# aszepieniec/stark-anatomy

Hardware: AMD Instinct MI355X
Metric: ntt_field_elements_per_sec (higher is better)
Workload: dtype u128; 1 GPU; ntt_fwd_inv_2^20_1gpu; log2n=20, parallelism=single, passes_per_transform=2

## Files before the change

stark-anatomy_amd/csrc/core.h:

```cpp
#pragma once
#include <hip/hip_runtime.h>
#include <dlfcn.h>
#include <cstdio>
#include <cstdlib>
#include <cstring>
#include <algorithm>
#include <atomic>
#include <chrono>
#include <cerrno>
#include <thread>
#include <sys/random.h>
#include <deque>
#include <functional>
#include <future>
#include <map>
#include <mutex>
#include <string>
#include <tuple>
#include <vector>

#pragma GCC visibility push(default)
#include "../../include/starkcore.h"
#pragma GCC visibility pop
#include "ntt_plan.h"
// ... 40 lines not shown
    void* p = nullptr;
    size_t bytes = 0;
};

struct PlanKey {
    int logn;
    uint64_t lo, hi;
    bool operator<(const PlanKey& o) const { return std::tie(logn, lo, hi) < std::tie(o.logn, o.lo, o.hi); }
};
struct PlanTables {
    Fe* mt = nullptr;
    int mt_log = 0;
    Fe* tl = nullptr;
    Fe* th = nullptr;
    Fe* th_ninv = nullptr;
    struct Direct { int logA, logR; bool scaled; Fe* d; };
    std::vector<Direct> direct;
    uint64_t last_use = 0;
};
struct OuterKey {
    uint64_t lo, hi, order, len, batch, col_base;
    int ninv;
    bool operator<(const OuterKey& o) const { return std::tie(lo, hi, order, len, batch, col_base, ninv) < std::tie(o.lo, o.hi, o.order, o.len, o.batch, o.col_base, o.ninv); }
};
struct OuterTable {
    Fe* d = nullptr;
    uint64_t last_use = 0;
};
struct PowKey {
    uint64_t lo, hi, hi_count;
    bool operator<(const PowKey& o) const { return std::tie(lo, hi, hi_count) < std::tie(o.lo, o.hi, o.hi_count); }
// ... 3 lines not shown
    Fe* hi = nullptr;
    uint64_t last_use = 0;
};

struct Ctx {
    bool init = false;
    int device = -1;
    hipStream_t stream = nullptr;
    std::string err;
    NttTuning tuning;
    std::map<PlanKey, PlanTables> plans;
    std::map<PowKey, PowTables> pows;
    std::map<OuterKey, OuterTable> outers;
    uint64_t tick = 0;
    bool foreign_streams = false;
    int small_divisor_direct = 1;
    std::vector<hipStream_t> seen_streams;
    DevBuf scratch[8];
    std::map<hipStream_t, DevBuf> ntt_work;
    int num_cus = 256;
    int xcd_remap = 1;
    int fixed_shapes = 1;
    int prio_balance = -1;
    int wave_local = 1;
    unsigned long long* trace = nullptr;
    int forest_four_lane_wgs = 256;
    int merkle_big_nlev = 2;
    int fri_tail = -1;
    int fri_tail_stall = -1;
    size_t verify_stage_bytes = 64ull << 20;
// ... 17 lines not shown
        hipError_t _e = (expr);                                                                               \
        if (_e != hipSuccess) return fail(SC_ERR_HIP, std::string(#expr) + ": " + hipGetErrorString(_e));     \
    } while (0)

#define SCCHK(expr)              \
    do {                         \
        int _rc = (expr);        \
        if (_rc != SC_OK) return _rc; \
    } while (0)

struct NttOpts {
    uint64_t in_limit = ~0ull;
    const PowTables* coset = nullptr;
    uint32_t cols = 1;
    uint64_t col_stride_in = 0;
};

constexpr uint64_t FUSE_MAX_W = 1ull << 17;

enum BuildMode { BUILD_SYNC = 0, BUILD_ASYNC = 1, BUILD_NOROOT = 2 };

extern Ctx g;
extern std::mutex g_mu;
extern hipStream_t g_comm_stream_for_free;
extern std::future<void> g_rand_worker;
extern size_t g_rand_prefetched;
extern std::multimap<size_t, void*> g_pool;
extern size_t g_pool_bytes, g_pool_cap;
extern std::deque<PendingFree> g_pending;
extern std::vector<hipEvent_t> g_event_pool;

void reap_pending(bool block);
hipError_t pool_alloc(void** p, size_t bytes);
void pool_free(void* p, size_t bytes);
void pool_clear();
hipEvent_t event_get();
int fail(int code, const std::string& msg);
int ensure_init();
int grow_buffer(DevBuf& b, size_t bytes, void** out);
inline int scratch(int slot, size_t bytes, void** out) { return grow_buffer(g.scratch[slot], bytes, out); }
int check_root(Fe root, uint64_t n);
int build_pow_table(Fe** out, uint64_t count, Fe base_m, uint64_t step, Fe scale_m, hipStream_t st);
void free_plans();
int evict_outer_tables();
int get_plan(Fe root, int logn, bool need_ninv, hipStream_t st, PlanTables** out);
inline NttTables tables_of(const PlanTables& t) {
    NttTables tb;
    tb.mt = t.mt; tb.mt_log = t.mt_log; tb.tl = t.tl; tb.th = t.th;
    return tb;
}
int get_pow(Fe base, uint64_t count, hipStream_t st, PowTables** out);
int plan_batched_direct(NttPlanDesc& d, BatchKind kind, int loglen, int logbatch, PlanTables* pt, const Fe* in, Fe* work, Fe* out, BatchExtras ex, hipStream_t st, bool* ok);
int run_plan(NttPlanDesc& d, hipStream_t st);
int ntt_device(const Fe* d_in, Fe* d_out, int logn, Fe root, bool inverse_scale, const NttOpts& o, hipStream_t st);
Fe root_inverse(Fe root, uint64_t n);
int ntt_any(const Fe* d_in, Fe* d_out, uint64_t n, Fe root, bool inverse, const NttOpts& o, hipStream_t st);
int upload(void* d, const void* h, size_t bytes, hipStream_t st);
int download(void* h, const void* d, size_t bytes, hipStream_t st);
int pointwise_div_device(const Fe* a, const Fe* b, Fe* out, uint64_t n, hipStream_t st);
int pointwise_div_enqueue(const Fe* a, const Fe* b, Fe* out, uint64_t n, hipStream_t st, uint32_t* flag);
int gather_device(const Fe* v, const uint64_t* d_idx, uint64_t k, Fe* d_out, hipStream_t st);
int read_small_polled(const void* d_src, size_t bytes, hipStream_t st, void* host_out);

int merkle_climb(uint64_t* levels, uint64_t N, int lvl, hipStream_t st, volatile uint64_t* host = nullptr, uint64_t seq = 0, bool* published = nullptr);
int merkle_finish(uint64_t* levels, uint64_t width, hipStream_t st);
int root_slot_get();
int merkle_build_device(const Fe* d_elems, uint64_t N, uint8_t root_out[64], sc_merkle** tree, hipStream_t st, BuildMode mode = BUILD_SYNC, const FoldIn* fold = nullptr);
int merkle_root_wait(sc_merkle* t, bool from_free = false);
// ... 82 lines not shown
```

stark-anatomy_amd/csrc/core.hip:

```cpp
#include "core.h"


template <int LOGE> struct PassThreads { static constexpr int value = LOGE >= 4 ? 256 : (LOGE == 3 ? 512 : 1024); };

template <int LOGE>
__global__ void __launch_bounds__(PassThreads<LOGE>::value) ntt_pass_kernel(const PassParams P, uint32_t ntiles, int xcd_remap) {
    extern __shared__ __attribute__((aligned(16))) unsigned char smem_raw[];
    Fe* lds = reinterpret_cast<Fe*>(smem_raw);
    uint32_t wg = blockIdx.x, colbits = 0;
    if (P.col_enable) { colbits = (wg >> P.col_tiles_log) << P.col_tiles_log; wg -= colbits; }
    uint32_t tile = wg;
    if (xcd_remap) tile = (wg & 7u) * (ntiles >> 3) + (wg >> 3);
    tile |= colbits;
    Fe* tw = lds + (1u << (P.logR + P.logC));
    tile_twiddles_to_lds(P, P.logR, threadIdx.x, blockDim.x, tw);
    __syncthreads();
    const int nrounds = (P.logR + LOGE - 1) / LOGE;
    int sh = P.logR;
    for (int r = 0; r < nrounds; ++r) {
        const int s = (r == 0) ? (P.logR - LOGE * (nrounds - 1)) : LOGE;
        sh -= s;
        ntt_round_dispatch<LOGE>(P, s, sh, r == 0, tile, threadIdx.x, lds, tw);
        if (r + 1 < nrounds) __syncthreads();
    }
// ... 381 lines not shown
    return SC_OK;
}

int build_pow_table(Fe** out, uint64_t count, Fe base_m, uint64_t step, Fe scale_m, hipStream_t st) {
    if (count == 0) count = 1;
    HIPCHK(hipMalloc((void**)out, count * sizeof(Fe)));
    unsigned blocks = (unsigned)((count + 255) / 256);
    hipLaunchKernelGGL(pow_table_kernel, dim3(blocks), dim3(256), 0, st, *out, count, base_m, step, scale_m);
    HIPCHK(hipGetLastError());
    return SC_OK;
}

void free_plan_tables(PlanTables& t) {
    hipFree(t.mt); hipFree(t.tl); hipFree(t.th);
    if (t.th_ninv) hipFree(t.th_ninv);
    for (const PlanTables::Direct& e : t.direct) hipFree(e.d);
}

void free_plans() {
    for (auto& kv : g.plans) free_plan_tables(kv.second);
    g.plans.clear();
    for (auto& kv : g.pows) { hipFree(kv.second.lo); hipFree(kv.second.hi); }
    g.pows.clear();
    for (auto& kv : g.outers) hipFree(kv.second.d);
    g.outers.clear();
}

constexpr uint64_t PIN_WINDOW = 64;
constexpr size_t PLAN_CAP = 256, POW_CAP = 64;

template <class Map, class FreeFn>
int evict_tables(Map& m, size_t cap, FreeFn free_entry) {
    if (m.size() < cap) return SC_OK;
    std::vector<std::pair<uint64_t, typename Map::iterator>> old;
    for (auto it = m.begin(); it != m.end(); ++it)
        if (it->second.last_use + PIN_WINDOW < g.tick) old.emplace_back(it->second.last_use, it);
    if (old.empty()) return SC_OK;
    std::sort(old.begin(), old.end(), [](const auto& a, const auto& b) { return a.first < b.first; });
    size_t drop = cap / 4 ? cap / 4 : 1;
    if (drop > old.size()) drop = old.size();
    HIPCHK(hipDeviceSynchronize());
    for (size_t i = 0; i < drop; ++i) { free_entry(old[i].second->second); m.erase(old[i].second); }
    return SC_OK;
}

int get_plan(Fe root, int logn, bool need_ninv, hipStream_t st, PlanTables** out) {
    PlanKey key{logn, root.lo, root.hi};
    auto it = g.plans.find(key);
    bool built = false;
    ++g.tick;
    if (it == g.plans.end()) {
        SCCHK(evict_tables(g.plans, PLAN_CAP, free_plan_tables));
        const uint64_t n = 1ull << logn;
        Fe rm = to_mont(root);
        const TableSizes sz = table_sizes(logn);
        PlanTables t;
        t.mt_log = sz.mt_log;
        SCCHK(build_pow_table(&t.mt, sz.mt, rm, n >> sz.mt_log, fe_mont_one(), st));
        SCCHK(build_pow_table(&t.tl, sz.tl, rm, 1, fe_mont_one(), st));
        SCCHK(build_pow_table(&t.th, sz.th, rm, 4096, fe_mont_one(), st));
        it = g.plans.emplace(key, t).first;
        built = true;
    }
    if (need_ninv && !it->second.th_ninv) {
        const uint64_t n = 1ull << logn;
        Fe ninv_m = mont_inv(to_mont(Fe{n, 0}));
        SCCHK(build_pow_table(&it->second.th_ninv, table_sizes(logn).th, to_mont(root), 4096, ninv_m, st));
        built = true;
    }
    if (built) HIPCHK(hipStreamSynchronize(st));
    it->second.last_use = g.tick;
    *out = &it->second;
    return SC_OK;
}

int get_pow(Fe base, uint64_t count, hipStream_t st, PowTables** out) {
    uint64_t hi_count = (count >> 12) + 1;
    uint64_t hc = 1; while (hc < hi_count) hc <<= 1;
    PowKey key{base.lo, base.hi, hc};
    auto it = g.pows.find(key);
    ++g.tick;
    if (it == g.pows.end()) {
        SCCHK(evict_tables(g.pows, POW_CAP, [](PowTables& t) { hipFree(t.lo); hipFree(t.hi); }));
        Fe bm = to_mont(base);
        PowTables t;
        SCCHK(build_pow_table(&t.lo, 4096, bm, 1, fe_mont_one(), st));
        SCCHK(build_pow_table(&t.hi, hc, bm, 4096, fe_mont_one(), st));
        HIPCHK(hipStreamSynchronize(st));
        it = g.pows.emplace(key, t).first;
    }
    it->second.last_use = g.tick;
    *out = &it->second;
    return SC_OK;
}

int direct_twiddles(PlanTables* pt, const NttPlanDesc& d, int i, bool scaled, hipStream_t st, const Fe** out) {
    const DirectTable t = direct_table(d, i, scaled);
    *out = nullptr;
    if (t.logR + t.logB > g.tuning.direct_tw_max_log) return SC_OK;
    for (const PlanTables::Direct& e : pt->direct)
        if (e.logA == t.logA && e.logR == t.logR && e.scaled == t.scaled) { *out = e.d; return SC_OK; }
    const uint64_t count = 1ull << (t.logR + t.logB);
    Fe* p;
    HIPCHK(hipMalloc((void**)&p, count * sizeof(Fe)));
    pt->direct.push_back({t.logA, t.logR, t.scaled, p});
    hipLaunchKernelGGL(twiddle_table_kernel, dim3((unsigned)((count + 255) / 256)), dim3(256), 0, st, p, t.logB, count, 1ull << t.logA,
                       pt->tl, t.scaled ? pt->th_ninv : pt->th);
    HIPCHK(hipGetLastError());
    HIPCHK(hipStreamSynchronize(st));
    *out = p;
    return SC_OK;
}

int plan_batched_direct(NttPlanDesc& d, BatchKind kind, int loglen, int logbatch, PlanTables* pt, const Fe* in, Fe* work, Fe* out, BatchExtras ex, hipStream_t st, bool* ok) {
    const NttTables tb = tables_of(*pt);
    *ok = plan_batched(d, kind, loglen, logbatch, tb, in, work, out, g.tuning, ex);
    if (!*ok || d.npasses != 2) return SC_OK;
    SCCHK(direct_twiddles(pt, d, 0, false, st, &ex.inner_twd));
    if (ex.inner_twd) *ok = plan_batched(d, kind, loglen, logbatch, tb, in, work, out, g.tuning, ex);
    return SC_OK;
}

template <int LOGE>
void launch_pass(const NttPassDesc& pd, hipStream_t st) {
    int remap = (g.xcd_remap && pd.ntiles >= 16 && (pd.ntiles & 7u) == 0) ? 1 : 0;
    const PassKernel k = pass_kernel(pd, g.fixed_shapes != 0);
    if constexpr (LOGE == 2) {
        if (k.kind == PK_FIXED4) {
            const int lr = pd.p.logR, lc = pd.p.logC;
#define SC_LAUNCH_FIXED(LR, LC, TR, ALT) \
    hipLaunchKernelGGL((ntt_pass_kernel_fixed<2, LR, LC, TR, ALT>), dim3(pd.ntiles * pd.cols), dim3(pd.threads), pd.lds_bytes, st, pd.p, pd.ntiles, remap, g.wave_local)
#define SC_FIXED(LR, LC)                                                          \
            if (lr == LR && lc == LC) {                                           \
// ... 24 lines not shown
        d.pass[i].p.trace = g.trace ? g.trace + trace_off : nullptr;
        trace_off += (size_t)d.pass[i].ntiles * d.pass[i].cols * (d.pass[i].threads >> 6) * TRACE_STAMPS;
        switch (d.pass[i].loge) {
            case 1: launch_pass<1>(d.pass[i], st); break;
            case 2: launch_pass<2>(d.pass[i], st); break;
            case 3: launch_pass<3>(d.pass[i], st); break;
            case 4: launch_pass<4>(d.pass[i], st); break;
            default: return fail(SC_ERR_UNSUPPORTED, "bad loge");
        }
        HIPCHK(hipGetLastError());
    }
    return SC_OK;
}

int ntt_device(const Fe* d_in, Fe* d_out, int logn, Fe root, bool inverse_scale, const NttOpts& o, hipStream_t st) {
    PlanTables* pt;
    SCCHK(get_plan(root, logn, inverse_scale, st, &pt));
    const uint64_t n = 1ull << logn;
    const int m = plan_num_passes(logn, g.tuning);
    NttTables tb = tables_of(*pt);
    tb.th_scaled = (inverse_scale && m > 1) ? pt->th_ninv : nullptr;
    NttIo io;
    io.in = d_in; io.out = d_out; io.in_limit = o.in_limit; io.cols = o.cols; io.col_stride_in = o.col_stride_in;
    if (m > 1) { void* w; SCCHK(grow_buffer(g.ntt_work[st], n * o.cols * sizeof(Fe), &w)); io.work = (Fe*)w; }
    if (o.coset) { io.ol = o.coset->lo; io.oh = o.coset->hi; }
    if (inverse_scale && m == 1) { io.scale_last = true; io.scale = mont_inv(to_mont(Fe{n, 0})); }
    NttPlanDesc d;
    if (!plan_ntt(d, logn, tb, io, g.tuning)) return fail(SC_ERR_UNSUPPORTED, "unsupported transform length");
    if (d.npasses > 1) {
        bool any = false;
        for (int i = 0; i + 1 < d.npasses; ++i) {
            SCCHK(direct_twiddles(pt, d, i, inverse_scale, st, &tb.twd[i]));
            any |= tb.twd[i] != nullptr;
        }
        if (any && !plan_ntt(d, logn, tb, io, g.tuning)) return fail(SC_ERR_UNSUPPORTED, "unsupported transform length");
    }
    return run_plan(d, st);
}

Fe root_inverse(Fe root, uint64_t n) {
    return from_mont(mont_pow(to_mont(root), n - 1));
}

int ntt_any(const Fe* d_in, Fe* d_out, uint64_t n, Fe root, bool inverse, const NttOpts& o, hipStream_t st) {
    if (n <= 1) {
        if (n == 1 && d_in != d_out) HIPCHK(hipMemcpyAsync(d_out, d_in, sizeof(Fe), hipMemcpyDeviceToDevice, st));
        return SC_OK;
// ... 225 lines not shown
    else if (k == "min_tiles_log") g.tuning.min_tiles_log = value;
    else if (k == "single_pass_max_log") g.tuning.single_pass_max_log = value;
    else if (k == "max_digit_log") g.tuning.max_digit_log = value;
    else if (k == "direct_tw_max_log") g.tuning.direct_tw_max_log = value;
    else if (k == "xcd_remap") g.xcd_remap = value;
    else if (k == "fixed_shapes") g.fixed_shapes = value;
    else if (k == "wave_local") g.wave_local = value;
    else if (k == "prio_balance") g.prio_balance = value;
    else if (k == "loge_cols") g.tuning.loge_cols = value;
    else if (k == "tw_on_load") g.tuning.tw_on_load = value;
    else if (k == "prune") g.tuning.prune = value;
    else if (k == "merkle_big_nlev") g.merkle_big_nlev = value < 0 ? 0 : (value > 8 ? 8 : value);
    else if (k == "forest_four_lane_wgs") g.forest_four_lane_wgs = value < 0 ? 0 : value;
    else if (k == "fri_tail") g.fri_tail = value ? 1 : 0;
    else if (k == "small_divisor_direct") g.small_divisor_direct = value ? 1 : 0;
    else if (k == "verify_stage_kb") g.verify_stage_bytes = (size_t)(value < 16 ? 16 : value) << 10;
    else if (k == "fri_tail_stall") g.fri_tail_stall = value;
    else if (k == "pool_cap_mb") g_pool_cap = (size_t)(value < 0 ? 0 : value) << 20;
    else if (k == "pool_trim") {
        if (g.init) { (void)hipDeviceSynchronize(); reap_pending(true); pool_clear(); }
    }
    else return fail(SC_ERR_BAD_ARG, "unknown tuning key " + k);
    return SC_OK;
}

int sc_ntt_num_passes(uint64_t n) {
    std::lock_guard<std::mutex> lk(g_mu);
    if (n < 2 || !is_pow2(n)) return 0;
    return plan_num_passes(ilog2(n), g.tuning);
}
// ... 383 lines not shown
    SCCHK(get_pow(fe_from(factor), rows * row_len, st, &pw));
    const uint64_t cnt = rows * cols;
    hipLaunchKernelGGL(scale_slab_kernel, dim3((unsigned)((cnt + 255) / 256)), dim3(256), 0, st, (const Fe*)d_in, (Fe*)d_out, rows, ilog2(cols), row_len, col_base, pw->lo, pw->hi);
    HIPCHK(hipGetLastError());
    return SC_OK;
}

int sc_poly_mul(const void* a, uint64_t na, const void* b, uint64_t nb, const uint64_t root[2], uint64_t order, void* out, uint64_t n_out) {
    std::lock_guard<std::mutex> lk(g_mu);
    SCCHK(ensure_init());
    if (!is_pow2(order) || order < 2) return fail(SC_ERR_NOT_POW2, "cannot compute ntt of non-power-of-two sequence");
    if (na > order || nb > order || n_out > order || na == 0 || nb == 0) return fail(SC_ERR_BAD_ARG, "operand longer than the transform order");
    Fe rt = fe_from(root);
    SCCHK(check_root(rt, order));
    hipStream_t st = g.stream;
    void *da, *db, *dc;
    SCCHK(scratch(1, order * sizeof(Fe), &da));
    SCCHK(scratch(2, order * sizeof(Fe), &db));
    SCCHK(scratch(3, order * sizeof(Fe), &dc));
    const int logn = ilog2(order);
    NttOpts o;
    SCCHK(upload(dc, a, na * sizeof(Fe), st));
    o.in_limit = na;
    SCCHK(ntt_device((const Fe*)dc, (Fe*)da, logn, rt, false, o, st));
    SCCHK(upload(dc, b, nb * sizeof(Fe), st));
    o.in_limit = nb;
    SCCHK(ntt_device((const Fe*)dc, (Fe*)db, logn, rt, false, o, st));
    hipLaunchKernelGGL(pointwise_mul_kernel, dim3((unsigned)((order + 255) / 256)), dim3(256), 0, st, (const Fe*)da, (const Fe*)db, (Fe*)dc, order);
    HIPCHK(hipGetLastError());
    SCCHK(ntt_device((const Fe*)dc, (Fe*)da, logn, root_inverse(rt, order), true, NttOpts{}, st));
    return download(out, da, n_out * sizeof(Fe), st);
}

static int coset_divide_core(const Fe* d_a, uint64_t na, const Fe* d_b, uint64_t nb, Fe off, Fe rt, uint64_t order, Fe** full, hipStream_t st, uint32_t* zero_flag = nullptr) {
    void *da, *db, *dc;
// ... 217 lines not shown
```

stark-anatomy_amd/csrc/fourstep.hip:

```cpp
#include "core.h"

__global__ void __launch_bounds__(256) outer_table_kernel(Fe* out, uint64_t count, int logcols, uint64_t col_base, const Fe* __restrict__ tl, const Fe* __restrict__ th) {
    uint64_t i = (uint64_t)blockIdx.x * blockDim.x + threadIdx.x;
    if (i >= count) return;
    uint64_t r = i >> logcols, c = i & ((1ull << logcols) - 1);
    out[i] = pow2level(tl, th, r * (col_base + c));
}

__global__ void __launch_bounds__(256) twiddle_matrix_kernel(Fe* __restrict__ data, uint64_t rows, int logcols, uint64_t row_base, uint64_t col_base,
                                                             const Fe* __restrict__ tl, const Fe* __restrict__ th, int scale_enable, Fe scale_m) {
    uint64_t i = (uint64_t)blockIdx.x * blockDim.x + threadIdx.x;
    if (i >= (rows << logcols)) return;
    uint64_t r = i >> logcols, c = i & ((1ull << logcols) - 1);
    uint64_t e = (row_base + r) * (col_base + c);
    Fe t = pow2level(tl, th, e);
    if (scale_enable) t = mont_mul(t, scale_m);
    data[i] = mont_mul(data[i], t);
}

extern "C" {

struct BatchCall {
    const Fe* in = nullptr;
    Fe* out = nullptr;
// ... 35 lines not shown
    ex.diag_lo = c.diag_lo;
    ex.diag_n = c.diag_n;
    ex.block_out = c.block_out;
    ex.block_rows = c.block_rows;
    if (c.out_ld) {
        if (kind != 1 || c.out_ld < batch) return fail(SC_ERR_BAD_ARG, "an output leading dimension belongs to kind 1 and must be >= batch");
        ex.out_ld = c.out_ld;
    }
    if (c.outer) {
        const uint64_t outer_order = c.outer_order, outer_col_base = c.outer_col_base;
        if (!is_pow2(outer_order) || outer_order < len * batch) return fail(SC_ERR_BAD_ARG, "outer twiddle order too small");
        if ((len - 1) * (outer_col_base + batch - 1) >= outer_order) return fail(SC_ERR_BAD_ARG, "outer twiddle exponent out of range");
        Fe ort = c.outer_root;
        if (!c.roots_checked) SCCHK(check_root(ort, outer_order));
        PlanTables* po;
        SCCHK(get_plan(ort, ilog2(outer_order), c.outer_ninv, st, &po));
        ex.outer_tl = po->tl;
        ex.outer_th = c.outer_ninv ? po->th_ninv : po->th;
        ex.outer_col_base = outer_col_base;
        if (g.tuning.direct_tw_max_log > 0 && len * batch <= (1ull << g.tuning.direct_tw_max_log)) {
            OuterKey ok{ort.lo, ort.hi, outer_order, len, batch, outer_col_base, c.outer_ninv ? 1 : 0};
            ++g.tick;
            auto it = g.outers.find(ok);
            if (it == g.outers.end()) {
                SCCHK(evict_outer_tables());
                OuterTable t;
                const uint64_t count = len * batch;
                HIPCHK(hipMalloc((void**)&t.d, count * sizeof(Fe)));
                hipLaunchKernelGGL(outer_table_kernel, dim3((unsigned)((count + 255) / 256)), dim3(256), 0, st, t.d, count, logbatch, outer_col_base, ex.outer_tl, ex.outer_th);
                HIPCHK(hipGetLastError());
                HIPCHK(hipStreamSynchronize(st));
// ... 501 lines not shown
```

stark-anatomy_amd/csrc/geoseq.cuh:

```cuda
#pragma once
#include "field.cuh"
#include "ntt_tile.cuh"

namespace sc {

#define GS_INDEX() ((uint64_t)blockIdx.x * blockDim.x + threadIdx.x)

constexpr int GS_E = 8;
constexpr int GS_T = 256;
constexpr uint64_t GS_BLOCK = (uint64_t)GS_E * GS_T;

__global__ void __launch_bounds__(GS_T) gs_totals_kernel(const Fe* __restrict__ a, uint64_t n, Fe* __restrict__ tot) {
    __shared__ Fe lds[GS_T];
    const uint32_t t = threadIdx.x;
    const uint64_t base = (uint64_t)blockIdx.x * GS_BLOCK + (uint64_t)t * GS_E;
    Fe prod = fe_mont_one();
#pragma unroll
    for (int k = 0; k < GS_E; ++k)
        if (base + k < n) prod = mont_mul(prod, a[base + k]);
    lds[t] = prod;
    for (uint32_t s = GS_T / 2; s > 0; s >>= 1) {
        __syncthreads();
        if (t < s) lds[t] = mont_mul(lds[t], lds[t + s]);
    }
// ... 55 lines not shown
    else v = mont_mul(mont_mul(geo_S(rev, n, k), geo_S(rev, n, n - k)), mont_mul(k2_m, t_m[k]));
    v = from_mont(v);
    zr[k] = (k & 1) ? fe_neg(v) : v;
}

__global__ void __launch_bounds__(256) geo_from_mont_kernel(Fe* __restrict__ a, uint64_t n) {
    const uint64_t i = GS_INDEX();
    if (i < n) a[i] = from_mont(a[i]);
}

__global__ void __launch_bounds__(256) geo_mul_tab_kernel(const Fe* __restrict__ in, const Fe* __restrict__ tab_m, Fe* __restrict__ out, uint64_t n) {
    const uint64_t i = GS_INDEX();
    if (i < n) out[i] = mont_mul(in[i], tab_m[i]);
}

__global__ void __launch_bounds__(256) geo_corr_kernel(const Fe* __restrict__ A, const Fe* __restrict__ B, Fe* __restrict__ D, uint64_t M, Fe c_m2) {
    const uint64_t f = GS_INDEX();
    if (f >= M) return;
    D[f] = mont_mul(mont_mul(A[(M - f) & (M - 1)], B[f]), c_m2);
}

__global__ void __launch_bounds__(256) geo_eval_in_kernel(const Fe* __restrict__ p, uint64_t m, const Fe* __restrict__ clo, const Fe* __restrict__ chi, const Fe* __restrict__ tinv_m,
                                                         Fe* __restrict__ out) {
    const uint64_t j = GS_INDEX();
    if (j >= m) return;
    Fe v = mont_mul(p[j], tinv_m[j]);
    if (clo) v = mont_mul(v, pow2level(clo, chi, j));
    out[j] = v;
}

// ... 31 lines not shown
```

stark-anatomy_amd/csrc/ntt_plan.h:

```cpp
#pragma once
#include "ntt_tile.cuh"

namespace sc {

struct NttTuning {
    int max_tile_log = -1;
    int loge = 2;
    int max_col_log = -1;
    int min_tiles_log = 8;
    int single_pass_max_log = 11;
    int max_digit_log = -1;
    int direct_tw_max_log = 22;
    int tw_on_load = 0;
    int prune = 1;
    int loge_cols = 3;
};

inline NttTuning resolve_tuning(const NttTuning& in, int logn) {
    NttTuning t = in;
    const bool small = logn <= 20;
    if (t.max_digit_log < 0) t.max_digit_log = small ? 10 : 8;
    if (t.max_tile_log < 0) t.max_tile_log = small ? 12 : 11;
    if (t.max_col_log < 0) t.max_col_log = small ? 4 : 6;
    if (t.tw_on_load < 0) t.tw_on_load = 0;
// ... 26 lines not shown
    int digits[4] = {0, 0, 0, 0};
    NttPassDesc pass[4];
};

struct NttIo {
    const Fe* in = nullptr;
    Fe* work = nullptr;
    Fe* out = nullptr;
    uint64_t in_limit = ~0ull;
    const Fe* ol = nullptr;
    const Fe* oh = nullptr;
    bool scale_last = false;
    Fe scale = Fe{0, 0};
    uint32_t cols = 1;
    uint64_t col_stride_in = 0;
};

inline int plan_num_passes(int logn, const NttTuning& tu_in) {
    const NttTuning tu = resolve_tuning(tu_in, logn);
    if (logn <= tu.single_pass_max_log) return 1;
    const int m = (logn + tu.max_digit_log - 1) / tu.max_digit_log;
    return m < 2 ? 2 : m;
}


struct TableSizes {
    int mt_log;
    uint64_t mt, tl, th;
};
inline TableSizes table_sizes(int logn) {
// ... 72 lines not shown
    if (transposing && pd.p.logR <= loge) loge = pd.p.logR - 1;
    if (loge < 1) return false;
    pd.loge = loge;
    pd.threads = 1u << (logT - loge);
    pd.lds_bytes = ((uint32_t)sizeof(Fe) << logT) + tile_twiddle_bytes(pd.p.logR);
    return true;
}

inline bool plan_ntt(NttPlanDesc& d, int logn, const NttTables& tb, const NttIo& io, const NttTuning& tu_in) {
    if (logn < 1 || logn > 32) return false;
    NttTuning tu = resolve_tuning(tu_in, logn);
    d.logn = logn;
    const int m = plan_num_passes(logn, tu);
    if (m > 4) return false;
    if (io.cols < 1 || io.cols > 65536) return false;
    int cols_log = 0;
    while ((2u << cols_log) <= io.cols) ++cols_log;
    if (io.cols > 1 && logn <= 16) {
        if (tu_in.max_tile_log < 0) tu.max_tile_log = 11;
        if (tu_in.max_col_log < 0) tu.max_col_log = 6;
    }
    d.npasses = m;
    split_digits(d, logn, m);
    const uint64_t n = 1ull << logn;
    const int tile_cap = shrink_tile_cap(tu, d.digits[0], logn + cols_log);

    int logA = 0;
    for (int i = 0; i < m; ++i) {
        NttPassDesc& pd = d.pass[i];
        PassParams& p = pd.p;
// ... 47 lines not shown
        }
        logA += logR;
    }
    if (tu.prune && io.in_limit < n && m > 1) {
        const int logR = d.digits[0];
        const uint64_t B = n >> logR;
        const uint64_t rows_nz = (io.in_limit + B - 1) / B;
        int k = 0;
        while (k < logR - 1 && ((uint64_t)1 << (logR - k - 1)) >= rows_nz && rows_nz > 0) ++k;
        const int loge = d.pass[0].loge;
        const int nr = (logR + loge - 1) / loge;
        const int cap = (logR - loge * (nr - 1)) + (nr > 1 ? loge : 0);
        if (k > cap) k = cap;
        d.pass[0].p.prune_log = k;
    }
    if (tu.tw_on_load) {
        int logAi = 0;
        for (int i = 0; i + 1 < m; ++i) {
            if (tb.twd[i]) {
                d.pass[i].p.tw_enable = 0;
                d.pass[i].p.twd = nullptr;
                d.pass[i + 1].p.twd_in = tb.twd[i];
                d.pass[i + 1].p.twd_in_mask = (1ull << (logn - logAi)) - 1;
            }
            logAi += d.digits[i];
        }
    }
    return true;
}

// ... 152 lines not shown
```

stark-anatomy_amd/csrc/polytree_geo.hip:

```cpp
#include "core.h"
#include "polytree.cuh"
#include "geoseq.cuh"

namespace sci {


Fe canonical_root(int logn) {
    static Fe cache[120];
    static bool have[120] = {false};
    if (!have[logn]) {
        Fe r = to_mont(Fe{0xb5038f9c18f6f7d1ull, 0x4040fbed12ee470full});
        for (int i = 119; i > logn; --i) r = mont_mul(r, r);
        cache[logn] = from_mont(r);
        have[logn] = true;
    }
    return cache[logn];
}

Fe ninv_scaled(int logn, int j) {
    Fe c = from_mont(mont_inv(to_mont(Fe{1ull << logn, 0})));
    for (int i = 0; i < j; ++i) c = to_mont(c);
    return c;
}

// ... 204 lines not shown
    return SC_OK;
}

}


struct sc_geodomain {
    uint64_t n, M;
    int logM;
    Fe c, q, c_inv;
    bool unit;
    Fe* tinv_m;
    Fe* wden_m;
    Fe* Bf;
    Fe* ZRf;
    Fe* zr;
};

namespace {

int scan_products(Fe* a, uint64_t n, hipStream_t st) {
    if (n == 0) return SC_OK;
    const uint64_t nb = (n + GS_BLOCK - 1) / GS_BLOCK;
    if (nb == 1) {
        hipLaunchKernelGGL(gs_apply_kernel, dim3(1), dim3(GS_T), 0, st, a, n, (const Fe*)nullptr);
        HIPCHK(hipGetLastError());
        return SC_OK;
    }
    PoolTmpAsync tot;
    SCCHK(tot.get(nb * sizeof(Fe)));
    hipLaunchKernelGGL(gs_totals_kernel, dim3((unsigned)nb), dim3(GS_T), 0, st, (const Fe*)a, n, tot.fe());
    SCCHK(scan_products(tot.fe(), nb, st));
    hipLaunchKernelGGL(gs_apply_kernel, dim3((unsigned)nb), dim3(GS_T), 0, st, a, n, (const Fe*)tot.fe());
    HIPCHK(hipGetLastError());
    return SC_OK;
}

void geodomain_release(sc_geodomain* d) {
    if (!d) return;
    if (d->tinv_m) release_after_streams(d->tinv_m, d->n * sizeof(Fe));
    if (d->wden_m) release_after_streams(d->wden_m, d->n * sizeof(Fe));
    if (d->Bf) release_after_streams(d->Bf, d->M * sizeof(Fe));
    if (d->ZRf) release_after_streams(d->ZRf, d->M * sizeof(Fe));
    if (d->zr) release_after_streams(d->zr, (d->n + 1) * sizeof(Fe));
    delete d;
}

int geodomain_create(Fe c, Fe q, uint64_t n, sc_geodomain** out, hipStream_t st) {
    if (n < 2) return fail(SC_ERR_UNSUPPORTED, "a progression of fewer than two points");
    if (fe_ge_p(c) || fe_ge_p(q) || fe_is_zero(c) || fe_is_zero(q)) return fail(SC_ERR_UNSUPPORTED, "first point and ratio must be non-zero residues");
    const int logM = ilog2(2 * n - 1);
    if (logM > 28) return fail(SC_ERR_UNSUPPORTED, "progression too long");
    const uint64_t M = 1ull << logM;
    sc_geodomain* d = new sc_geodomain{n, M, logM, c, q, Fe{0, 0}, fe_eq(c, fe_one()), nullptr, nullptr, nullptr, nullptr, nullptr};
    auto bail = [&](int rc) { geodomain_release(d); return rc; };
    auto alloc = [&](Fe** p, uint64_t count) -> int {
        hipError_t e = pool_alloc((void**)p, count * sizeof(Fe));
        return e == hipSuccess ? SC_OK : fail(SC_ERR_HIP, hipGetErrorString(e));
    };
    int rc = alloc(&d->tinv_m, n);
    if (rc == SC_OK) rc = alloc(&d->wden_m, n);
    if (rc == SC_OK) rc = alloc(&d->Bf, M);
    if (rc == SC_OK) rc = alloc(&d->ZRf, M);
    if (rc == SC_OK) rc = alloc(&d->zr, n + 1);
    if (rc != SC_OK) return bail(rc);
    const Fe q_m = to_mont(q);
    const Fe qinv = from_mont(mont_inv(q_m));
    d->c_inv = from_mont(mont_inv(to_mont(c)));
    PoolTmpAsync tt, A, rev;
    if ((rc = tt.get(M * sizeof(Fe))) != SC_OK || (rc = A.get(n * sizeof(Fe))) != SC_OK || (rc = rev.get(n * sizeof(Fe))) != SC_OK) return bail(rc);
    PowTables *pq, *pqi, *pg;
    if ((rc = get_pow(q, M, st, &pq)) != SC_OK) return bail(rc);
    if ((rc = get_pow(qinv, n, st, &pqi)) != SC_OK) return bail(rc);
    hipLaunchKernelGGL(geo_fill_kernel, dim3(pt_blocks(M)), dim3(256), 0, st, tt.fe(), M, 0, n, (const Fe*)pq->lo, (const Fe*)pq->hi);
    if ((rc = scan_products(tt.fe(), M, st)) != SC_OK) return bail(rc);
    hipLaunchKernelGGL(geo_fill_kernel, dim3(pt_blocks(n)), dim3(256), 0, st, d->tinv_m, n, 0, n, (const Fe*)pqi->lo, (const Fe*)pqi->hi);
    if ((rc = scan_products(d->tinv_m, n, st)) != SC_OK) return bail(rc);
    hipLaunchKernelGGL(geo_fill_kernel, dim3(pt_blocks(n)), dim3(256), 0, st, A.fe(), n, 1, n, (const Fe*)pq->lo, (const Fe*)pq->hi);
    if ((rc = scan_products(A.fe(), n, st)) != SC_OK) return bail(rc);
    hipLaunchKernelGGL(geo_fill_kernel, dim3(pt_blocks(n - 1)), dim3(256), 0, st, rev.fe(), n - 1, 2, n, (const Fe*)pq->lo, (const Fe*)pq->hi);
// ... 5 lines not shown
    if (fe_is_zero(an1_m)) return bail(fail(SC_ERR_UNSUPPORTED, "the points of the progression are not distinct"));
    const Fe ia_m = mont_inv(an1_m);
    const Fe k1_m = mont_mul(ia_m, ia_m);
    const Fe k2_m = mont_mul(an_m, k1_m);
    const Fe g = from_mont(mont_pow(to_mont(qinv), n - 2));
    if ((rc = get_pow(g, n, st, &pg)) != SC_OK) return bail(rc);
    hipLaunchKernelGGL(geo_wden_kernel, dim3(pt_blocks(n)), dim3(256), 0, st, d->wden_m, n, (const Fe*)rev.fe(), k1_m, (const Fe*)pg->lo, (const Fe*)pg->hi);
    hipLaunchKernelGGL(geo_zr_kernel, dim3(pt_blocks(n + 1)), dim3(256), 0, st, d->zr, n, (const Fe*)rev.fe(), (const Fe*)tt.fe(), k2_m);
    hipLaunchKernelGGL(geo_from_mont_kernel, dim3(pt_blocks(M)), dim3(256), 0, st, tt.fe(), M);
    if (hipGetLastError() != hipSuccess) return bail(fail(SC_ERR_HIP, "progression table launch failed"));
    const Fe rt = canonical_root(logM);
    if ((rc = ntt_device(tt.fe(), d->Bf, logM, rt, false, NttOpts(), st)) != SC_OK) return bail(rc);
    NttOpts o;
    o.in_limit = n;
    if ((rc = ntt_device(d->zr, d->ZRf, logM, rt, false, o, st)) != SC_OK) return bail(rc);
    *out = d;
    return SC_OK;
}

const PowTables* geo_cpow(const sc_geodomain* d, Fe base, uint64_t count, hipStream_t st, int* rc) {
    if (d->unit) { *rc = SC_OK; return nullptr; }
    PowTables* pw = nullptr;
    *rc = get_pow(base, count, st, &pw);
    return pw;
}

int geodomain_evaluate_chunk(const sc_geodomain* d, const Fe* p, uint64_t len, Fe* dst, Fe* bx, Fe* by, hipStream_t st) {
    const uint64_t n = d->n, M = d->M;
    if (len == 0) { HIPCHK(hipMemsetAsync(dst, 0, n * sizeof(Fe), st)); return SC_OK; }
    int rc;
    const PowTables* pc = geo_cpow(d, d->c, n, st, &rc);
    SCCHK(rc);
    hipLaunchKernelGGL(geo_eval_in_kernel, dim3(pt_blocks(len)), dim3(256), 0, st, p, len, pc ? (const Fe*)pc->lo : nullptr, pc ? (const Fe*)pc->hi : nullptr, (const Fe*)d->tinv_m, bx);
    const Fe rt = canonical_root(d->logM);
    NttOpts o;
    o.in_limit = len;
    SCCHK(ntt_device(bx, by, d->logM, rt, false, o, st));
    hipLaunchKernelGGL(geo_corr_kernel, dim3(pt_blocks(M)), dim3(256), 0, st, (const Fe*)by, (const Fe*)d->Bf, bx, M, ninv_scaled(d->logM, 2));
    SCCHK(ntt_device(bx, by, d->logM, root_inverse(rt, M), false, NttOpts(), st));
    hipLaunchKernelGGL(geo_mul_tab_kernel, dim3(pt_blocks(n)), dim3(256), 0, st, (const Fe*)by, (const Fe*)d->tinv_m, dst, n);
    HIPCHK(hipGetLastError());
    return SC_OK;
}

int geodomain_evaluate(const sc_geodomain* d, const Fe* coeffs, uint64_t m, Fe* out, hipStream_t st) {
    const uint64_t n = d->n, M = d->M;
    PoolTmpAsync bx, by;
// ... 51 lines not shown
    return rc;
}

int geodomain_interpolate(const sc_geodomain* d, const Fe* values, Fe* out, hipStream_t st) {
    const uint64_t n = d->n, M = d->M;
    PoolTmpAsync bx, by;
    SCCHK(bx.get(M * sizeof(Fe)));
    SCCHK(by.get(M * sizeof(Fe)));
    int rc;
    const PowTables* pi = geo_cpow(d, d->c_inv, n, st, &rc);
    SCCHK(rc);
    const Fe rt = canonical_root(d->logM), rti = root_inverse(rt, M);
    const Fe c_m2 = ninv_scaled(d->logM, 2);
    NttOpts o;
    o.in_limit = n;
    hipLaunchKernelGGL(geo_mul_tab_kernel, dim3(pt_blocks(n)), dim3(256), 0, st, values, (const Fe*)d->wden_m, bx.fe(), n);
    SCCHK(ntt_device(bx.fe(), by.fe(), d->logM, rt, false, o, st));
    hipLaunchKernelGGL(geo_corr_kernel, dim3(pt_blocks(M)), dim3(256), 0, st, (const Fe*)by.fe(), (const Fe*)d->Bf, bx.fe(), M, c_m2);
    SCCHK(ntt_device(bx.fe(), by.fe(), d->logM, rti, false, NttOpts(), st));
    hipLaunchKernelGGL(geo_mul_tab_kernel, dim3(pt_blocks(n)), dim3(256), 0, st, (const Fe*)by.fe(), (const Fe*)d->tinv_m, bx.fe(), n);
    SCCHK(ntt_device(bx.fe(), by.fe(), d->logM, rt, false, o, st));
    hipLaunchKernelGGL(pt_mul_scaled_kernel, dim3(pt_blocks(M)), dim3(256), 0, st, (const Fe*)by.fe(), (const Fe*)d->ZRf, bx.fe(), M, c_m2);
    SCCHK(ntt_device(bx.fe(), by.fe(), d->logM, rti, false, NttOpts(), st));
    hipLaunchKernelGGL(geo_rev_scale_kernel, dim3(pt_blocks(n)), dim3(256), 0, st, (const Fe*)by.fe(), n, pi ? (const Fe*)pi->lo : nullptr, pi ? (const Fe*)pi->hi : nullptr, out);
    HIPCHK(hipGetLastError());
    return SC_OK;
}

}

// ... 216 lines not shown
```

Before: 44.63 billion field-elements/s.

## Fuse pointwise multiplies into NTT first-pass loads for multiply and geo-domain paths

Adds a mul_in operand to the NTT plan so the first pass multiplies its input by a table on load. Polynomial multiply and the geometric-domain evaluate/interpolate use this in place of separate pointwise kernels. Polynomial multiply also runs both forward transforms as one two-column NTT and folds the canonical operand into an extra n^-1·R scaled twiddle table. This cuts kernel launches and global memory round trips, at the cost of extra precomputed tables and added plan complexity. The benchmarked plain forward/inverse NTT probably does not touch these paths.

```diff
diff --git a/stark-anatomy_amd/csrc/core.h b/stark-anatomy_amd/csrc/core.h
--- a/stark-anatomy_amd/csrc/core.h
+++ b/stark-anatomy_amd/csrc/core.h
@@ -78,7 +78,8 @@
     Fe* tl = nullptr;
     Fe* th = nullptr;
     Fe* th_ninv = nullptr;
-    struct Direct { int logA, logR; bool scaled; Fe* d; };
+    Fe* th_ninv_r = nullptr;
+    struct Direct { int logA, logR; int scaled; Fe* d; };
     std::vector<Direct> direct;
     uint64_t last_use = 0;
 };
@@ -112,6 +113,7 @@
     std::map<OuterKey, OuterTable> outers;
     uint64_t tick = 0;
     bool foreign_streams = false;
+    int fuse_pointwise = 1;
     int small_divisor_direct = 1;
     std::vector<hipStream_t> seen_streams;
     DevBuf scratch[8];
@@ -159,7 +161,11 @@
     const PowTables* coset = nullptr;
     uint32_t cols = 1;
     uint64_t col_stride_in = 0;
-};
+    const Fe* mul_in = nullptr;
+    bool mul_in_canonical = false;
+};
+enum { SCALE_NONE = 0, SCALE_NINV = 1, SCALE_NINV_R = 2 };
+
 
 constexpr uint64_t FUSE_MAX_W = 1ull << 17;
 
@@ -188,7 +194,7 @@
 int build_pow_table(Fe** out, uint64_t count, Fe base_m, uint64_t step, Fe scale_m, hipStream_t st);
 void free_plans();
 int evict_outer_tables();
-int get_plan(Fe root, int logn, bool need_ninv, hipStream_t st, PlanTables** out);
+int get_plan(Fe root, int logn, int need_scale, hipStream_t st, PlanTables** out);
 inline NttTables tables_of(const PlanTables& t) {
     NttTables tb;
     tb.mt = t.mt; tb.mt_log = t.mt_log; tb.tl = t.tl; tb.th = t.th;
@@ -197,6 +203,7 @@
 int get_pow(Fe base, uint64_t count, hipStream_t st, PowTables** out);
 int plan_batched_direct(NttPlanDesc& d, BatchKind kind, int loglen, int logbatch, PlanTables* pt, const Fe* in, Fe* work, Fe* out, BatchExtras ex, hipStream_t st, bool* ok);
 int run_plan(NttPlanDesc& d, hipStream_t st);
+inline bool fuse_pointwise() { return g.fuse_pointwise && !g.tuning.tw_on_load; }
 int ntt_device(const Fe* d_in, Fe* d_out, int logn, Fe root, bool inverse_scale, const NttOpts& o, hipStream_t st);
 Fe root_inverse(Fe root, uint64_t n);
 int ntt_any(const Fe* d_in, Fe* d_out, uint64_t n, Fe root, bool inverse, const NttOpts& o, hipStream_t st);
diff --git a/stark-anatomy_amd/csrc/core.hip b/stark-anatomy_amd/csrc/core.hip
--- a/stark-anatomy_amd/csrc/core.hip
+++ b/stark-anatomy_amd/csrc/core.hip
@@ -419,6 +419,7 @@
 void free_plan_tables(PlanTables& t) {
     hipFree(t.mt); hipFree(t.tl); hipFree(t.th);
     if (t.th_ninv) hipFree(t.th_ninv);
+    if (t.th_ninv_r) hipFree(t.th_ninv_r);
     for (const PlanTables::Direct& e : t.direct) hipFree(e.d);
 }
 
@@ -449,7 +450,7 @@
     return SC_OK;
 }
 
-int get_plan(Fe root, int logn, bool need_ninv, hipStream_t st, PlanTables** out) {
+int get_plan(Fe root, int logn, int need_scale, hipStream_t st, PlanTables** out) {
     PlanKey key{logn, root.lo, root.hi};
     auto it = g.plans.find(key);
     bool built = false;
@@ -467,10 +468,16 @@
         it = g.plans.emplace(key, t).first;
         built = true;
     }
-    if (need_ninv && !it->second.th_ninv) {
+    if (need_scale == SCALE_NINV && !it->second.th_ninv) {
         const uint64_t n = 1ull << logn;
         Fe ninv_m = mont_inv(to_mont(Fe{n, 0}));
         SCCHK(build_pow_table(&it->second.th_ninv, table_sizes(logn).th, to_mont(root), 4096, ninv_m, st));
+        built = true;
+    }
+    if (need_scale == SCALE_NINV_R && !it->second.th_ninv_r) {
+        const uint64_t n = 1ull << logn;
+        Fe ninv_r_m = to_mont(mont_inv(to_mont(Fe{n, 0})));
+        SCCHK(build_pow_table(&it->second.th_ninv_r, table_sizes(logn).th, to_mont(root), 4096, ninv_r_m, st));
         built = true;
     }
     if (built) HIPCHK(hipStreamSynchronize(st));
@@ -499,18 +506,19 @@
     return SC_OK;
 }
 
-int direct_twiddles(PlanTables* pt, const NttPlanDesc& d, int i, bool scaled, hipStream_t st, const Fe** out) {
-    const DirectTable t = direct_table(d, i, scaled);
+int direct_twiddles(PlanTables* pt, const NttPlanDesc& d, int i, int scaled, hipStream_t st, const Fe** out) {
+    const DirectTable t = direct_table(d, i, scaled != SCALE_NONE);
+    const int kind = t.scaled ? scaled : SCALE_NONE;
     *out = nullptr;
     if (t.logR + t.logB > g.tuning.direct_tw_max_log) return SC_OK;
     for (const PlanTables::Direct& e : pt->direct)
-        if (e.logA == t.logA && e.logR == t.logR && e.scaled == t.scaled) { *out = e.d; return SC_OK; }
+        if (e.logA == t.logA && e.logR == t.logR && e.scaled == kind) { *out = e.d; return SC_OK; }
     const uint64_t count = 1ull << (t.logR + t.logB);
     Fe* p;
     HIPCHK(hipMalloc((void**)&p, count * sizeof(Fe)));
-    pt->direct.push_back({t.logA, t.logR, t.scaled, p});
+    pt->direct.push_back({t.logA, t.logR, kind, p});
     hipLaunchKernelGGL(twiddle_table_kernel, dim3((unsigned)((count + 255) / 256)), dim3(256), 0, st, p, t.logB, count, 1ull << t.logA,
-                       pt->tl, t.scaled ? pt->th_ninv : pt->th);
+                       pt->tl, kind == SCALE_NINV_R ? pt->th_ninv_r : kind == SCALE_NINV ? pt->th_ninv : pt->th);
     HIPCHK(hipGetLastError());
     HIPCHK(hipStreamSynchronize(st));
     *out = p;
@@ -521,7 +529,7 @@
     const NttTables tb = tables_of(*pt);
     *ok = plan_batched(d, kind, loglen, logbatch, tb, in, work, out, g.tuning, ex);
     if (!*ok || d.npasses != 2) return SC_OK;
-    SCCHK(direct_twiddles(pt, d, 0, false, st, &ex.inner_twd));
+    SCCHK(direct_twiddles(pt, d, 0, SCALE_NONE, st, &ex.inner_twd));
     if (ex.inner_twd) *ok = plan_batched(d, kind, loglen, logbatch, tb, in, work, out, g.tuning, ex);
     return SC_OK;
 }
@@ -576,23 +584,27 @@
 }
 
 int ntt_device(const Fe* d_in, Fe* d_out, int logn, Fe root, bool inverse_scale, const NttOpts& o, hipStream_t st) {
+    if (o.mul_in_canonical && !(o.mul_in && inverse_scale)) return fail(SC_ERR_UNSUPPORTED, "a canonical operand on load needs an inverse transform to absorb its 2^-128");
+    const int scaled = !inverse_scale ? SCALE_NONE : o.mul_in_canonical ? SCALE_NINV_R : SCALE_NINV;
     PlanTables* pt;
-    SCCHK(get_plan(root, logn, inverse_scale, st, &pt));
+    SCCHK(get_plan(root, logn, scaled, st, &pt));
     const uint64_t n = 1ull << logn;
     const int m = plan_num_passes(logn, g.tuning);
     NttTables tb = tables_of(*pt);
-    tb.th_scaled = (inverse_scale && m > 1) ? pt->th_ninv : nullptr;
+    tb.th_scaled = (inverse_scale && m > 1) ? (scaled == SCALE_NINV_R ? pt->th_ninv_r : pt->th_ninv) : nullptr;
     NttIo io;
     io.in = d_in; io.out = d_out; io.in_limit = o.in_limit; io.cols = o.cols; io.col_stride_in = o.col_stride_in;
+    io.mul_in = o.mul_in;
     if (m > 1) { void* w; SCCHK(grow_buffer(g.ntt_work[st], n * o.cols * sizeof(Fe), &w)); io.work = (Fe*)w; }
     if (o.coset) { io.ol = o.coset->lo; io.oh = o.coset->hi; }
     if (inverse_scale && m == 1) { io.scale_last = true; io.scale = mont_inv(to_mont(Fe{n, 0})); }
+    if (scaled == SCALE_NINV_R && m == 1) io.scale = to_mont(io.scale);
     NttPlanDesc d;
     if (!plan_ntt(d, logn, tb, io, g.tuning)) return fail(SC_ERR_UNSUPPORTED, "unsupported transform length");
     if (d.npasses > 1) {
         bool any = false;
         for (int i = 0; i + 1 < d.npasses; ++i) {
-            SCCHK(direct_twiddles(pt, d, i, inverse_scale, st, &tb.twd[i]));
+            SCCHK(direct_twiddles(pt, d, i, scaled, st, &tb.twd[i]));
             any |= tb.twd[i] != nullptr;
         }
         if (any && !plan_ntt(d, logn, tb, io, g.tuning)) return fail(SC_ERR_UNSUPPORTED, "unsupported transform length");
@@ -848,6 +860,7 @@
     else if (k == "forest_four_lane_wgs") g.forest_four_lane_wgs = value < 0 ? 0 : value;
     else if (k == "fri_tail") g.fri_tail = value ? 1 : 0;
     else if (k == "small_divisor_direct") g.small_divisor_direct = value ? 1 : 0;
+    else if (k == "fuse_pointwise") g.fuse_pointwise = value ? 1 : 0;
     else if (k == "verify_stage_kb") g.verify_stage_bytes = (size_t)(value < 16 ? 16 : value) << 10;
     else if (k == "fri_tail_stall") g.fri_tail_stall = value;
     else if (k == "pool_cap_mb") g_pool_cap = (size_t)(value < 0 ? 0 : value) << 20;
@@ -1261,11 +1274,31 @@
     Fe rt = fe_from(root);
     SCCHK(check_root(rt, order));
     hipStream_t st = g.stream;
+    const int logn = ilog2(order);
+    if (fuse_pointwise()) {
+        const uint64_t L = na > nb ? na : nb;
+        void *stage, *spec, *res;
+        SCCHK(scratch(3, 2 * L * sizeof(Fe), &stage));
+        SCCHK(scratch(1, 2 * order * sizeof(Fe), &spec));
+        SCCHK(scratch(2, order * sizeof(Fe), &res));
+        if (na != nb) HIPCHK(hipMemsetAsync(stage, 0, 2 * L * sizeof(Fe), st));
+        SCCHK(upload(stage, a, na * sizeof(Fe), st));
+        SCCHK(upload((Fe*)stage + L, b, nb * sizeof(Fe), st));
+        NttOpts o;
+        o.in_limit = L;
+        o.cols = 2;
+        o.col_stride_in = L;
+        SCCHK(ntt_device((const Fe*)stage, (Fe*)spec, logn, rt, false, o, st));
+        NttOpts oi;
+        oi.mul_in = (const Fe*)spec + order;
+        oi.mul_in_canonical = true;
+        SCCHK(ntt_device((const Fe*)spec, (Fe*)res, logn, root_inverse(rt, order), true, oi, st));
+        return download(out, res, n_out * sizeof(Fe), st);
+    }
     void *da, *db, *dc;
     SCCHK(scratch(1, order * sizeof(Fe), &da));
     SCCHK(scratch(2, order * sizeof(Fe), &db));
     SCCHK(scratch(3, order * sizeof(Fe), &dc));
-    const int logn = ilog2(order);
     NttOpts o;
     SCCHK(upload(dc, a, na * sizeof(Fe), st));
     o.in_limit = na;
diff --git a/stark-anatomy_amd/csrc/fourstep.hip b/stark-anatomy_amd/csrc/fourstep.hip
--- a/stark-anatomy_amd/csrc/fourstep.hip
+++ b/stark-anatomy_amd/csrc/fourstep.hip
@@ -73,7 +73,7 @@
         Fe ort = c.outer_root;
         if (!c.roots_checked) SCCHK(check_root(ort, outer_order));
         PlanTables* po;
-        SCCHK(get_plan(ort, ilog2(outer_order), c.outer_ninv, st, &po));
+        SCCHK(get_plan(ort, ilog2(outer_order), c.outer_ninv ? SCALE_NINV : SCALE_NONE, st, &po));
         ex.outer_tl = po->tl;
         ex.outer_th = c.outer_ninv ? po->th_ninv : po->th;
         ex.outer_col_base = outer_col_base;
diff --git a/stark-anatomy_amd/csrc/geoseq.cuh b/stark-anatomy_amd/csrc/geoseq.cuh
--- a/stark-anatomy_amd/csrc/geoseq.cuh
+++ b/stark-anatomy_amd/csrc/geoseq.cuh
@@ -93,6 +93,11 @@
     if (i < n) out[i] = mont_mul(in[i], tab_m[i]);
 }
 
+__global__ void __launch_bounds__(256) geo_operand_kernel(const Fe* __restrict__ tab, Fe* __restrict__ out, uint64_t M, Fe k_m2) {
+    const uint64_t f = GS_INDEX();
+    if (f < M) out[f] = mont_mul(tab[f], k_m2);
+}
+
 __global__ void __launch_bounds__(256) geo_corr_kernel(const Fe* __restrict__ A, const Fe* __restrict__ B, Fe* __restrict__ D, uint64_t M, Fe c_m2) {
     const uint64_t f = GS_INDEX();
     if (f >= M) return;
diff --git a/stark-anatomy_amd/csrc/ntt_plan.h b/stark-anatomy_amd/csrc/ntt_plan.h
--- a/stark-anatomy_amd/csrc/ntt_plan.h
+++ b/stark-anatomy_amd/csrc/ntt_plan.h
@@ -64,6 +64,7 @@
     Fe scale = Fe{0, 0};
     uint32_t cols = 1;
     uint64_t col_stride_in = 0;
+    const Fe* mul_in = nullptr;
 };
 
 inline int plan_num_passes(int logn, const NttTuning& tu_in) {
@@ -166,6 +167,7 @@
     const int m = plan_num_passes(logn, tu);
     if (m > 4) return false;
     if (io.cols < 1 || io.cols > 65536) return false;
+    if (io.mul_in && tu.tw_on_load) return false;
     int cols_log = 0;
     while ((2u << cols_log) <= io.cols) ++cols_log;
     if (io.cols > 1 && logn <= 16) {
@@ -243,6 +245,10 @@
         if (k > cap) k = cap;
         d.pass[0].p.prune_log = k;
     }
+    if (io.mul_in) {
+        d.pass[0].p.twd_in = io.mul_in;
+        d.pass[0].p.twd_in_mask = n - 1;
+    }
     if (tu.tw_on_load) {
         int logAi = 0;
         for (int i = 0; i + 1 < m; ++i) {
diff --git a/stark-anatomy_amd/csrc/polytree_geo.hip b/stark-anatomy_amd/csrc/polytree_geo.hip
--- a/stark-anatomy_amd/csrc/polytree_geo.hip
+++ b/stark-anatomy_amd/csrc/polytree_geo.hip
@@ -242,6 +242,8 @@
     Fe* wden_m;
     Fe* Bf;
     Fe* ZRf;
+    Fe* Bf_op;
+    Fe* ZRf_op;
     Fe* zr;
 };
 
@@ -266,10 +268,12 @@
 
 void geodomain_release(sc_geodomain* d) {
     if (!d) return;
-    if (d->tinv_m) release_after_streams(d->tinv_m, d->n * sizeof(Fe));
-    if (d->wden_m) release_after_streams(d->wden_m, d->n * sizeof(Fe));
+    if (d->tinv_m) release_after_streams(d->tinv_m, d->M * sizeof(Fe));
+    if (d->wden_m) release_after_streams(d->wden_m, d->M * sizeof(Fe));
     if (d->Bf) release_after_streams(d->Bf, d->M * sizeof(Fe));
     if (d->ZRf) release_after_streams(d->ZRf, d->M * sizeof(Fe));
+    if (d->Bf_op) release_after_streams(d->Bf_op, d->M * sizeof(Fe));
+    if (d->ZRf_op) release_after_streams(d->ZRf_op, d->M * sizeof(Fe));
     if (d->zr) release_after_streams(d->zr, (d->n + 1) * sizeof(Fe));
     delete d;
 }
@@ -280,18 +284,22 @@
     const int logM = ilog2(2 * n - 1);
     if (logM > 28) return fail(SC_ERR_UNSUPPORTED, "progression too long");
     const uint64_t M = 1ull << logM;
-    sc_geodomain* d = new sc_geodomain{n, M, logM, c, q, Fe{0, 0}, fe_eq(c, fe_one()), nullptr, nullptr, nullptr, nullptr, nullptr};
+    sc_geodomain* d = new sc_geodomain{n, M, logM, c, q, Fe{0, 0}, fe_eq(c, fe_one()), nullptr, nullptr, nullptr, nullptr, nullptr, nullptr, nullptr};
     auto bail = [&](int rc) { geodomain_release(d); return rc; };
     auto alloc = [&](Fe** p, uint64_t count) -> int {
         hipError_t e = pool_alloc((void**)p, count * sizeof(Fe));
         return e == hipSuccess ? SC_OK : fail(SC_ERR_HIP, hipGetErrorString(e));
     };
-    int rc = alloc(&d->tinv_m, n);
-    if (rc == SC_OK) rc = alloc(&d->wden_m, n);
+    int rc = alloc(&d->tinv_m, M);
+    if (rc == SC_OK) rc = alloc(&d->wden_m, M);
     if (rc == SC_OK) rc = alloc(&d->Bf, M);
     if (rc == SC_OK) rc = alloc(&d->ZRf, M);
+    if (rc == SC_OK) rc = alloc(&d->Bf_op, M);
+    if (rc == SC_OK) rc = alloc(&d->ZRf_op, M);
     if (rc == SC_OK) rc = alloc(&d->zr, n + 1);
     if (rc != SC_OK) return bail(rc);
+    if (hipMemsetAsync(d->tinv_m + n, 0, (M - n) * sizeof(Fe), st) != hipSuccess || hipMemsetAsync(d->wden_m + n, 0, (M - n) * sizeof(Fe), st) != hipSuccess)
+        return bail(fail(SC_ERR_HIP, "clearing the progression tables failed"));
     const Fe q_m = to_mont(q);
     const Fe qinv = from_mont(mont_inv(q_m));
     d->c_inv = from_mont(mont_inv(to_mont(c)));
@@ -327,6 +335,10 @@
     NttOpts o;
     o.in_limit = n;
     if ((rc = ntt_device(d->zr, d->ZRf, logM, rt, false, o, st)) != SC_OK) return bail(rc);
+    const Fe c_m2 = ninv_scaled(logM, 2);
+    hipLaunchKernelGGL(geo_operand_kernel, dim3(pt_blocks(M)), dim3(256), 0, st, (const Fe*)d->Bf, d->Bf_op, M, c_m2);
+    hipLaunchKernelGGL(geo_operand_kernel, dim3(pt_blocks(M)), dim3(256), 0, st, (const Fe*)d->ZRf, d->ZRf_op, M, c_m2);
+    if (hipGetLastError() != hipSuccess) return bail(fail(SC_ERR_HIP, "progression operand launch failed"));
     *out = d;
     return SC_OK;
 }
@@ -344,6 +356,20 @@
     int rc;
     const PowTables* pc = geo_cpow(d, d->c, n, st, &rc);
     SCCHK(rc);
+    if (fuse_pointwise()) {
+        const Fe rti = root_inverse(canonical_root(d->logM), M);
+        NttOpts o;
+        o.in_limit = len;
+        o.coset = pc;
+        o.mul_in = d->tinv_m;
+        SCCHK(ntt_device(p, by, d->logM, rti, false, o, st));
+        NttOpts oc;
+        oc.mul_in = d->Bf_op;
+        SCCHK(ntt_device(by, bx, d->logM, rti, false, oc, st));
+        hipLaunchKernelGGL(geo_mul_tab_kernel, dim3(pt_blocks(n)), dim3(256), 0, st, (const Fe*)bx, (const Fe*)d->tinv_m, dst, n);
+        HIPCHK(hipGetLastError());
+        return SC_OK;
+    }
     hipLaunchKernelGGL(geo_eval_in_kernel, dim3(pt_blocks(len)), dim3(256), 0, st, p, len, pc ? (const Fe*)pc->lo : nullptr, pc ? (const Fe*)pc->hi : nullptr, (const Fe*)d->tinv_m, bx);
     const Fe rt = canonical_root(d->logM);
     NttOpts o;
@@ -425,6 +451,20 @@
     const Fe c_m2 = ninv_scaled(d->logM, 2);
     NttOpts o;
     o.in_limit = n;
+    if (fuse_pointwise()) {
+        NttOpts ow = o, oc, ot = o, oz;
+        ow.mul_in = d->wden_m;
+        oc.mul_in = d->Bf_op;
+        ot.mul_in = d->tinv_m;
+        oz.mul_in = d->ZRf_op;
+        SCCHK(ntt_device(values, by.fe(), d->logM, rti, false, ow, st));
+        SCCHK(ntt_device(by.fe(), bx.fe(), d->logM, rti, false, oc, st));
+        SCCHK(ntt_device(bx.fe(), by.fe(), d->logM, rt, false, ot, st));
+        SCCHK(ntt_device(by.fe(), bx.fe(), d->logM, rti, false, oz, st));
+        hipLaunchKernelGGL(geo_rev_scale_kernel, dim3(pt_blocks(n)), dim3(256), 0, st, (const Fe*)bx.fe(), n, pi ? (const Fe*)pi->lo : nullptr, pi ? (const Fe*)pi->hi : nullptr, out);
+        HIPCHK(hipGetLastError());
+        return SC_OK;
+    }
     hipLaunchKernelGGL(geo_mul_tab_kernel, dim3(pt_blocks(n)), dim3(256), 0, st, values, (const Fe*)d->wden_m, bx.fe(), n);
     SCCHK(ntt_device(bx.fe(), by.fe(), d->logM, rt, false, o, st));
     hipLaunchKernelGGL(geo_corr_kernel, dim3(pt_blocks(M)), dim3(256), 0, st, (const Fe*)by.fe(), (const Fe*)d->Bf, bx.fe(), M, c_m2);
```

Result: no change. 44.65 billion field-elements/s, median of 3 (+0.0%).
